# jambo6/online-neural-cdes

Hardware: AMD Instinct MI355X
Metric: solved integration steps/sec (fwd+adjoint) (higher is better)
Workload: dtype f32; 1 GPU; BASELINE cfg2: rectilinear interpolation, rk4 step 1, B=4096 per GPU (global 4096), raw L=200 -> T=399 knots, C=20, H=HH=32, nl=3; step = forward + adjoint backward + Adam; global_batch=4096, seq_len=200, parallelism=dp1

## Files before the change

include/ncde_hip.h:

```cpp
#ifndef NCDE_HIP_H
#define NCDE_HIP_H

#include <stddef.h>
#include <stdint.h>

#ifdef __cplusplus
extern "C" {
#endif

#define NCDE_ABI_VERSION 4
#define NCDE_MAX_LAYERS 8

typedef enum NcdeStatus {
    NCDE_OK = 0,
    NCDE_ERR_INVALID = -1,
    NCDE_ERR_UNSUPPORTED = -2,
    NCDE_ERR_WORKSPACE = -3,
    NCDE_ERR_HIP = -4
} NcdeStatus;

typedef enum NcdeInterp { NCDE_INTERP_LINEAR = 0, NCDE_INTERP_CUBIC = 1, NCDE_INTERP_QUINTIC = 2 } NcdeInterp;

typedef enum NcdeMethod { NCDE_EULER = 0, NCDE_MIDPOINT = 1, NCDE_RK4_38 = 2 } NcdeMethod;

typedef enum NcdeOutput { NCDE_OUT_INTERVAL = 0, NCDE_OUT_KNOTS = 1, NCDE_OUT_TIMES = 2 } NcdeOutput;

#define NCDE_FLAG_AUTO 0u
#define NCDE_FLAG_FORCE_GENERIC 1u
#define NCDE_FLAG_FORCE_FAST 2u
#define NCDE_FLAG_FP32_MFMA 4u
#define NCDE_FLAG_ADJOINT_V1 8u
#define NCDE_FLAG_ADJOINT_V2 16u
#define NCDE_FLAG_ADJOINT_V4 32u
#define NCDE_FLAG_SPLIT_BF16 64u
#define NCDE_FLAG_ADJOINT_SPLIT_FP16 128u
#define NCDE_FLAG_DEBUG_PROFILE 0x100u
#define NCDE_FLAG_NO_COOP 0x400u
#define NCDE_FLAG_COOP_FAULT_INJECT 0x800u
#define NCDE_FLAG_TILED_NS1 0x1000u
#define NCDE_FLAG_TILED_NS2 0x2000u
#define NCDE_FLAG_TILED_NS4 0x4000u
#define NCDE_FLAG_FORCE_TILED 0x8000u

#define NCDE_FLAG_TILED_WINDOW_STEPS(n) (((uint32_t)(n) & 0xFFu) << 16)

typedef struct NcdeProblem {
    int32_t abi_version;
    int32_t batch;
    int32_t n_knots;
    int32_t channels;
    int32_t hidden;
    int32_t interp;
    int32_t method;
    int32_t output;
    uint32_t flags;

    int32_t n_layers;
    int32_t layer_in[NCDE_MAX_LAYERS];
    int32_t layer_out[NCDE_MAX_LAYERS];
    const float* layer_W[NCDE_MAX_LAYERS];
    const float* layer_b[NCDE_MAX_LAYERS];
    const float* Wo;
    const float* bo;

    const float* coeffs;
    int64_t coeffs_stride_b;
    int64_t coeffs_stride_t;

    const float* z0;

    int32_t field_kind;
    int32_t field_input;
    const float* Wg;
    const float* bg;
    const float* Wr;
    const float* br;

    const void* time_plan;
    int32_t n_t_out;
    int32_t n_steps_fwd;
    int32_t n_steps_adj;
    int32_t reserved_;
} NcdeProblem;

typedef enum NcdeFieldKind { NCDE_FIELD_ORIGINAL = 0, NCDE_FIELD_MINIMAL = 1, NCDE_FIELD_GRU = 2 } NcdeFieldKind;
typedef enum NcdeFieldInput { NCDE_INPUT_MATMUL = 0, NCDE_INPUT_EVALUATE = 1, NCDE_INPUT_DERIVATIVE = 2 } NcdeFieldInput;

typedef struct NcdeGrads {
    float* grad_z0;
    float* grad_layer_W[NCDE_MAX_LAYERS];
    float* grad_layer_b[NCDE_MAX_LAYERS];
    float* grad_Wo;
    float* grad_bo;
    float* grad_Wg;
    float* grad_bg;
// ... 102 lines not shown
```

online-neural-cdes_amd/_lib.py:

```python
import ctypes
import os

NCDE_ABI_VERSION = 4
NCDE_MAX_LAYERS = 8

INTERP = {"linear": 0, "cubic": 1, "quintic": 2}
INTERP_PARTS = {"linear": 1, "cubic": 4, "quintic": 6}
METHOD = {"euler": 0, "midpoint": 1, "rk4": 2}
OUT_INTERVAL, OUT_KNOTS, OUT_TIMES = 0, 1, 2
FIELD_KIND = {"original": 0, "minimal": 1, "gru": 2}
FIELD_INPUT = {"matmul": 0, "evaluate": 1, "derivative": 2}
FLAG_AUTO, FLAG_FORCE_GENERIC, FLAG_FORCE_FAST, FLAG_FP32_MFMA, FLAG_ADJOINT_V1, FLAG_ADJOINT_V2 = 0, 1, 2, 4, 8, 16
FLAG_ADJOINT_V4 = 32
FLAG_SPLIT_BF16 = 64
FLAG_NO_COOP = 0x400
FLAG_COOP_FAULT_INJECT = 0x800
FLAG_ADJOINT_SPLIT_FP16 = 128


def FLAG_TILED_WINDOW_STEPS(n):
    return (int(n) & 0xFF) << 16
FLAG_TILED_NS1, FLAG_TILED_NS2, FLAG_TILED_NS4, FLAG_FORCE_TILED = 0x1000, 0x2000, 0x4000, 0x8000

_c_float_p = ctypes.c_void_p


class NcdeProblem(ctypes.Structure):
    _fields_ = [
        ("abi_version", ctypes.c_int32),
        ("batch", ctypes.c_int32),
        ("n_knots", ctypes.c_int32),
        ("channels", ctypes.c_int32),
        ("hidden", ctypes.c_int32),
        ("interp", ctypes.c_int32),
        ("method", ctypes.c_int32),
        ("output", ctypes.c_int32),
        ("flags", ctypes.c_uint32),
        ("n_layers", ctypes.c_int32),
        ("layer_in", ctypes.c_int32 * NCDE_MAX_LAYERS),
        ("layer_out", ctypes.c_int32 * NCDE_MAX_LAYERS),
        ("layer_W", _c_float_p * NCDE_MAX_LAYERS),
        ("layer_b", _c_float_p * NCDE_MAX_LAYERS),
        ("Wo", _c_float_p),
        ("bo", _c_float_p),
        ("coeffs", _c_float_p),
        ("coeffs_stride_b", ctypes.c_int64),
        ("coeffs_stride_t", ctypes.c_int64),
        ("z0", _c_float_p),
        ("field_kind", ctypes.c_int32),
        ("field_input", ctypes.c_int32),
        ("Wg", _c_float_p),
        ("bg", _c_float_p),
        ("Wr", _c_float_p),
        ("br", _c_float_p),
        ("time_plan", ctypes.c_void_p),
        ("n_t_out", ctypes.c_int32),
        ("n_steps_fwd", ctypes.c_int32),
        ("n_steps_adj", ctypes.c_int32),
        ("reserved_", ctypes.c_int32),
    ]


class NcdeTimeSpec(ctypes.Structure):
    _fields_ = [
        ("n_t", ctypes.c_int32),
        ("time_is_f64", ctypes.c_int32),
        ("t", ctypes.POINTER(ctypes.c_double)),
        ("step_size", ctypes.c_double),
        ("knots", ctypes.POINTER(ctypes.c_double)),
    ]


class NcdeTimePlanInfo(ctypes.Structure):
    _fields_ = [
        ("n_t_out", ctypes.c_int32),
# ... 156 lines not shown
```

online-neural-cdes_amd/csrc/ncde_common.h:

```cpp
#pragma once
#include <hip/hip_runtime.h>
#include <stdint.h>

#include "ncde_hip.h"

typedef float f32x4 __attribute__((ext_vector_type(4)));

__device__ __forceinline__ float quintic_eval(const float* p, int cs, float f, bool value) {
    const float bb = p[cs], c2 = p[2 * cs], d3 = p[3 * cs], e4 = p[4 * cs], f5 = p[5 * cs];
    if (value) {
        float inner = 0.25f * e4 + (f5 * f) / 5.0f;
        inner = d3 / 3.0f + inner * f;
        inner = 0.5f * c2 + inner * f;
        inner = bb + inner * f;
        return p[0] + inner * f;
    }
    float inner = e4 + f5 * f;
    inner = d3 + inner * f;
    inner = c2 + inner * f;
    return bb + inner * f;
}

#define NCDE_TILE 16

// ... 7 lines not shown
    const float* coeffs;
    long long cs_b, cs_t;
    const float* z0;
    float* out;
    const float* z_out;
    const float* grad_out;
    float* grad_z0;
    float* gpart;
    int gW_off[NCDE_MAX_LAYERS], gb_off[NCDE_MAX_LAYERS];
    int gWo_off, gbo_off, theta_size;
    int gacc_in_lds;
    float* stages;
    int discrete;
    float* recA;
    float* recB;
    float* recC;
    float* recD;
    int gstride;
    int win_hi, win_lo, resume;
    float* carry;
    int field_kind, field_input;
    int d0;
    int rows;
    const float* Wg;
    const float* bg;
    const float* Wr;
    const float* br;
    int gWg_off, gbg_off, gWr_off, gbr_off;
    const int* plan;
    int n_steps_fwd, n_steps_adj;
    const float* Wo_pk;
    int* fault;
    int only_faulted;
    const float* Wg_pk;
    const unsigned* Wo_bf;
    int wres[NCDE_MAX_LAYERS], wres_o, wres_g, wres_r;
    int tres[NCDE_MAX_LAYERS], tres_o, tres_g;
    int Hr, Cc;
    const unsigned* coop_img;
    float* coop_x;
    float* coop_state;
    unsigned* coop_sync;
    const float* coop_scale;
    int coop_M, coop_G;
    float* recS;
    unsigned* win_max;
    int dw2_parts;
    int dw2_accum;
    int Brec;
    unsigned* coop_status;
    const unsigned* run_if;
    unsigned coop_spin;
    int coop_inject;
};

typedef void (*NcdeKernel)(KArgs);

#define NCDE_PLAN_MAGIC 0x4e43504c
#define NCDE_PLAN_HEADER 8
struct StageDesc {
    int idx;
    float frac;
    float kdt;
};
__host__ __device__ __forceinline__ int plan_step_words(int S) { return 3 + 3 * S; }
__host__ __device__ __forceinline__ int plan_off_fwd() { return NCDE_PLAN_HEADER; }
__host__ __device__ __forceinline__ int plan_off_out(int S, int n_fwd) { return NCDE_PLAN_HEADER + n_fwd * plan_step_words(S); }
__host__ __device__ __forceinline__ int plan_off_adj(int S, int n_fwd, int n_out) { return plan_off_out(S, n_fwd) + 2 * n_out; }
__device__ __forceinline__ bool plan_header_ok(const KArgs& a, int S) {
    const int* h = a.plan;
    return h[0] == NCDE_PLAN_MAGIC && h[1] == S && h[2] == a.n_steps_fwd && h[3] == a.n_steps_adj && h[4] == a.n_out;
}
__device__ __forceinline__ StageDesc plan_stage(const int* step, int j) {
    StageDesc d;
    d.idx = step[3 + 3 * j];
    d.frac = __int_as_float(step[4 + 3 * j]);
    d.kdt = __int_as_float(step[5 + 3 * j]);
    return d;
}

__device__ __forceinline__ int ru4(int x) { return (x + 3) & ~3; }
__device__ __forceinline__ int ru16(int x) { return (x + 15) & ~15; }

__device__ __forceinline__ f32x4 mfma16(float a, float b, f32x4 c) {
    return __builtin_amdgcn_mfma_f32_16x16x4f32(a, b, c, 0, 0, 0);
}

__device__ __forceinline__ float tanh_dev(float x) {
    const float e = __builtin_amdgcn_exp2f(x * 2.8853900817779268f);
    const float r = __builtin_amdgcn_rcpf(e + 1.0f);
    return __builtin_fmaf(-2.0f, r, 1.0f);
}

#define NCDE_TANH_PRESCALE 2.8853900817779268f
__device__ __forceinline__ float tanh_prescaled(float x2l) {
    const float e = __builtin_amdgcn_exp2f(x2l);
    const float r = __builtin_amdgcn_rcpf(e + 1.0f);
    return __builtin_fmaf(-2.0f, r, 1.0f);
}

__device__ __forceinline__ float relu_dev(float x) { return __builtin_amdgcn_fmed3f(x, 0.0f, __builtin_inff()); }

__device__ __forceinline__ int n_stages(int method) { return method == NCDE_RK4_38 ? 4 : (method == NCDE_MIDPOINT ? 2 : 1); }
__device__ __forceinline__ float stage_offset(int method, int j) {
    if (method == NCDE_RK4_38) return j == 0 ? 0.0f : (j == 1 ? 0.333333343267440796f : (j == 2 ? 0.666666686534881592f : 1.0f));
    if (method == NCDE_MIDPOINT) return j == 0 ? 0.0f : 0.5f;
// ... 67 lines not shown
```

online-neural-cdes_amd/csrc/ncde_fast.hip:

```cpp
#include "ncde_fast.h"
#include "ncde_fast4.h"
#include "ncde_fast64.h"
#include "ncde_fast_nl.h"
#include "ncde_fast_c.h"
#include "ncde_fast_fwd3.h"
#include "ncde_fast_plan.h"
#ifndef NCDE_F2_DW_LATE
#define NCDE_F2_DW_LATE 0
#endif
#ifndef NCDE_F2_DXL_BF3
#define NCDE_F2_DXL_BF3 1
#endif
#ifndef NCDE_F2_DWO_EARLY
#define NCDE_F2_DWO_EARLY 0
#endif
#ifndef NCDE_H2_DW_LATE
#define NCDE_H2_DW_LATE 1
#endif
#ifndef NCDE_H2_DWO_EARLY
#define NCDE_H2_DWO_EARLY 0
#endif

#include <cstring>
#include <type_traits>
// ... 1610 lines not shown
    unsigned long long prof[6] = {0, 0, 0, 0, 0, 0}, tlast = 0;
#define NCDE_TICK(k)                                                \
    if constexpr (PROF != 0) {                                      \
        const unsigned long long now_ = __builtin_readcyclecounter(); \
        prof[k] += now_ - tlast;                                    \
        tlast = now_;                                               \
    }
    constexpr int H = 32, HH = 32, NW = 4, HT = 2;
    constexpr int CP = (C + 3) & ~3, CQ = CP / 4, NB = H / 4 / NW;
    constexpr int S = kStages<METHOD>;
    constexpr int NT = 64 * NW;
    constexpr int DXW = INTERP == NCDE_INTERP_LINEAR ? CP : 3 * CP;
    constexpr int EPT = (16 * DXW + NT - 1) / NT;
    constexpr int NTILE = NB * CQ, NBLK = NTILE / 2;
    constexpr int XROWS = H + NL * HH;
    constexpr int NFLAG = NTILE + 2;
    constexpr int HPF = HP != 0 ? 1 : 0, HPC = HP == 1 ? 1 : 0;
    typedef SplitOps<HPF> SF;
    typedef SplitOps<HPC> SO;
    typedef typename SF::T SpF;
    typedef typename SO::T SpT;
    constexpr int NPF = SF::NP, NP = SO::NP;
    if constexpr (HP == 0) {
        if (a.only_faulted && a.fault[blockIdx.x] == 0) return;
    }
    static_assert(NB == 2 && NTILE % 2 == 0, "one 32-row dWo block per cq");
    static_assert(PLAN == 0 || DISC == 0, "the planned discrete backward runs on the batch-tiled family");
    if constexpr (PLAN != 0) {
        if (a.plan == nullptr || !plan_header_ok(a, S)) return;
    }
    const int pw_ = plan_step_words(S);
    const int* padj = PLAN ? a.plan + plan_off_adj(S, a.n_steps_fwd, a.n_out) : nullptr;
    const int n_rsteps = PLAN ? a.n_steps_adj : a.T - 1;
    extern __shared__ __attribute__((aligned(16))) float lds[];
    float* zx = lds;
    float* dxs = zx + 2 * H * 16;
    constexpr int DXR = PLAN ? 2 * S * 16 * CP : 3 * 16 * DXW;
    float* red = dxs + DXR;
    float* boL = red + NW * HH * 16;
    float* tiles = boL + NW * NTILE * 16;
    float* ximg = tiles + NW * NTILE * 256;
    float* dpimg = ximg + 2 * XROWS * 16;
    constexpr int NDP = ((HP == 1 && NCDE_H2_DW_LATE != 0) || (HP == 2 && NCDE_F2_DW_LATE != 0 && INTERP == NCDE_INTERP_LINEAR)) ? 2 : 1;
    constexpr bool DXL3 = HP == 2 && NCDE_F2_DXL_BF3 != 0;
    constexpr bool DWO0_LATE = (HP == 1 && NCDE_H2_DWO_EARLY == 0) || (HP == 2 && NCDE_F2_DWO_EARLY == 0);
    int* flags = reinterpret_cast<int*>(dpimg + NDP * NL * HH * 16);
    float* biasL = reinterpret_cast<float*>(flags + NW * NFLAG);
    unsigned* w1T3 = reinterpret_cast<unsigned*>(biasL + 2 * HT * 16);
    unsigned* w0T3 = w1T3 + HT * NP * 256;
    unsigned* woLo = w0T3 + NW * NP * 256;
    unsigned* w1S3 = woLo + ((HP == 2 && !DXL3) ? 0 : NW * NB * CQ * 256);
    float* amax = reinterpret_cast<float*>(w1S3 + 2 * HT * NPF * 256);
    int* fault_s = reinterpret_cast<int*>(amax + NW);
    float mx = 0.0f;
    float sig = 1.0f;

    const int tid = threadIdx.x, lane = tid & 63;
    const int wave = __builtin_amdgcn_readfirstlane(tid >> 6);
    const bool is_chain = wave < NW;
    const int pw = is_chain ? wave : wave - NW;
    const int s = lane & 15, g = lane >> 4;
    const int b0 = blockIdx.x * NCDE_TILE;
    const int bs = b0 + s;
    const bool valid = bs < a.B;
    float* my_tiles = tiles + pw * NTILE * 256;
    volatile __attribute__((address_space(3))) int* my_flags =
        (volatile __attribute__((address_space(3))) int*)(flags + pw * NFLAG);
    volatile __attribute__((address_space(3))) int* xflag = (volatile __attribute__((address_space(3))) int*)(flags + NTILE);
    const float* boLw = boL + pw * NTILE * 16;

    for (int e = tid; e < NW * NFLAG; e += 512) flags[e] = 0;
    if (tid == 0) *fault_s = 0;
    for (int e = tid; e < NW * NTILE * 16; e += 512) {
        const int r = e & 3, gg = (e >> 2) & 3, rest = e >> 4;
        const int t2 = rest % NTILE, wv = rest / NTILE;
        const int nb = t2 / CQ, cq = t2 - nb * CQ;
        const int h = 4 * (wv * NB + nb) + gg, c = 4 * cq + r;
        boL[e] = c < C ? NCDE_TANH_PRESCALE * a.bo[h * C + c] : 0.0f;
    }
    for (int e = tid; e < 2 * HT * 16; e += 512) {
        const int r = e & 3, gg = (e >> 2) & 3, t = (e >> 4) % HT, layer = e / (16 * HT);
        biasL[e] = (layer == 0 || NL > 1) ? a.b[layer][8 * gg + 4 * t + r] : 0.0f;
    }
    if (tid < 64 * HT) {
        const int l = tid & 63, t = tid >> 6;
        const int unit_out = 8 * ((l & 15) >> 2) + 4 * t + (l & 3);
        float tmp[8];
#pragma unroll
        for (int jj = 0; jj < 8; ++jj) tmp[jj] = NL > 1 ? a.W[1][(8 * (l >> 4) + jj) * HH + unit_out] : 0.0f;
        SO::store(w1T3 + t * NP * 256, l, SO::split(tmp, mx));
    } else if (tid >= 64 * HT + 64 * NW && tid < 64 * HT + 64 * NW + 64 * HT) {
        const int l = tid & 63, t = (tid >> 6) - HT - NW;
        const int unitA = 8 * ((l & 15) >> 2) + 4 * t + (l & 3);
#pragma unroll
        for (int layer = 0; layer < 2; ++layer) {
            float tmp[8];
#pragma unroll
            for (int jj = 0; jj < 8; ++jj) tmp[jj] = (layer == 0 || NL > 1) ? a.W[layer][unitA * HH + 8 * (l >> 4) + jj] : 0.0f;
            SF::store(w1S3 + (layer * HT + t) * NPF * 256, l, SF::split(tmp, mx));
        }
    } else if (tid < 64 * HT + 64 * NW) {
        const int l = tid & 63, wv = (tid >> 6) - HT;
        const int r_own = l & 3;
        const int hrow = 4 * (wv * NB + r_own) + ((l & 15) >> 2);
        float tmp[8];
#pragma unroll
// ... 3 lines not shown

    if (is_chain) {
        u32x4 woHi[NB][CQ], woMid[NB][CQ];
        unsigned* my_woLo = woLo + pw * NB * CQ * 256;
        auto fwd_weights = [&](int layer, int tt) { return SF::load(w1S3 + (layer * HT + tt) * NPF * 256, lane); };
        auto wo_operand = [&](int nb, int cq) {
            SpF As;
            As.hi = woHi[nb][cq];
            if constexpr (HPF != 0) {
                As.lo = woMid[nb][cq];
            } else {
                As.mid = woMid[nb][cq];
                As.lo = *reinterpret_cast<const u32x4*>(my_woLo + ((nb * CQ + cq) * 64 + lane) * 4);
            }
            return As;
        };
#pragma unroll
        for (int nb = 0; nb < NB; ++nb)
#pragma unroll
            for (int cq = 0; cq < CQ; ++cq) {
                const int hA = 4 * (pw * NB + nb) + (s >> 2), cA = 4 * cq + (s & 3);
                float tmp[8];
#pragma unroll
                for (int jj = 0; jj < 8; ++jj) tmp[jj] = cA < C ? NCDE_TANH_PRESCALE * a.Wo[(hA * C + cA) * HH + 8 * g + jj] : 0.0f;
                const SpF sp = SF::split(tmp, mx);
                woHi[nb][cq] = sp.hi;
                if constexpr (HPF != 0) {
                    woMid[nb][cq] = sp.lo;
                } else {
                    woMid[nb][cq] = sp.mid;
                    *reinterpret_cast<u32x4*>(my_woLo + ((nb * CQ + cq) * 64 + lane) * 4) = sp.lo;
                }
            }
        const float* eptr[EPT];
        float eprev[EPT], enext[EPT];
        bool eok[EPT];
#pragma unroll
        for (int q = 0; q < EPT; ++q) {
            const int e = tid + q * NT;
            const int es = e / DXW, ec = e - es * DXW;
            const int part = ec / CP, c = ec - part * CP;
            eok[q] = e < 16 * DXW && c < a.Cc && (b0 + es) < a.B;
            const long long base = (long long)(eok[q] ? b0 + es : 0) * a.cs_b;
            eptr[q] = a.coeffs + base + (INTERP == NCDE_INTERP_LINEAR ? c : (part + 1) * a.Cc + c);
            eprev[q] = 0.0f;
            enext[q] = 0.0f;
        }
        auto stage_load = [&](int piece) {
#pragma unroll
            for (int q = 0; q < EPT; ++q) enext[q] = eok[q] ? eptr[q][(long long)piece * a.cs_t] : 0.0f;
        };
        auto stage_store = [&](int piece) {
            float* dst = dxs + (piece % 3) * 16 * DXW;
#pragma unroll
            for (int q = 0; q < EPT; ++q) {
                const int e = tid + q * NT;
                if (e < 16 * DXW) dst[e] = INTERP == NCDE_INTERP_LINEAR ? eprev[q] - enext[q] : enext[q];
                eprev[q] = enext[q];
            }
        };
        constexpr int EPQ = PLAN ? (S * 16 * CP + NT - 1) / NT : 1;
        float qn[EPQ];
        auto plan_load = [&](const int* pstep) {
#pragma unroll
            for (int q = 0; q < EPQ; ++q) {
                const int e = tid + q * NT;
                const int j = e / (16 * CP), rem = e - j * (16 * CP), es = rem / CP, c = rem - es * CP;
                float v = 0.0f;
                if (e < S * 16 * CP && c < a.Cc && b0 + es < a.B) {
                    const StageDesc sd = plan_stage(pstep, j);
                    const float* p = a.coeffs + (long long)(b0 + es) * a.cs_b + (long long)sd.idx * a.cs_t;
                    if constexpr (INTERP == NCDE_INTERP_LINEAR) {
                        v = p[a.cs_t + c] - p[c];
                        if (sd.kdt != 1.0f) v = v / sd.kdt;
                    } else {
                        const float bb = p[a.Cc + c], cc = p[2 * a.Cc + c], dd = p[3 * a.Cc + c];
                        const float inner = cc + dd * sd.frac;
                        v = bb + inner * sd.frac;
                    }
                }
                qn[q] = v;
            }
        };
        auto plan_store = [&](int buf) {
#pragma unroll
            for (int q = 0; q < EPQ; ++q) {
                const int e = tid + q * NT;
                if (e < S * 16 * CP) dxs[buf * (S * 16 * CP) + e] = qn[q];
            }
        };
        const int p_hi = a.n_pieces - 1;
        if constexpr (PLAN != 0) {
            plan_load(padj);
            plan_store(0);
        } else {
            if (INTERP == NCDE_INTERP_LINEAR) {
#pragma unroll
                for (int q = 0; q < EPT; ++q) eprev[q] = eok[q] ? eptr[q][(long long)(p_hi + 1) * a.cs_t] : 0.0f;
            }
            stage_load(p_hi);
            stage_store(p_hi);
            if (p_hi >= 1) {
                stage_load(p_hi - 1);
                stage_store(p_hi - 1);
            }
        }
        const int last_row = a.n_out - 1;
        float y0[NB], ky1[NB], ky2[NB], a0[NB], ka1[NB], ka2[NB], as_[NB], zreg[8];
        f32x4 znext[2];
        auto rec_fetch = [&](int lin) {
            const float* rp = a.stages + ((long long)lin * a.B + (valid ? bs : 0)) * a.Hr + 8 * g;
// ... 490 lines not shown
                        Aw.lo = *reinterpret_cast<const u32x4*>(my_woTlo + (((t_lo / 2) * HT + tt) * 64 + lane) * 4);
                        mfma_split2(Aw, Bq, accJ[tt], accJx[tt]);
                    }
                }
            } else {
                float bq[t_hi - t_lo][4];
#pragma unroll
                for (int tau = t_lo; tau < t_hi; ++tau)
#pragma unroll
                    for (int r = 0; r < 4; ++r) bq[tau - t_lo][r] = my_tiles[tau * 256 + (4 * g + r) * 16 + s];
#pragma unroll
                for (int tau = t_lo; tau < t_hi; ++tau)
#pragma unroll
                    for (int tt = 0; tt < HT; ++tt)
#pragma unroll
                        for (int r = 0; r < 4; ++r) accJ[tt] = mfma16(woT[tau][tt][r], bq[tau - t_lo][r], accJ[tt]);
            }
        };
        auto rescale_acc = [&]() {
            if constexpr (HPC != 0) {
                if (sig != acc_sig) {
                    const float ratio = sig * h2_inv_scale(acc_sig);
#pragma unroll
                    for (int i = 0; i < NBLK; ++i) {
                        gbo[i] *= ratio;
#pragma unroll
                        for (int q = 0; q < 16; ++q) gWo[i][q] *= ratio;
                    }
#pragma unroll
                    for (int r = 0; r < 4; ++r) { gW1[r] *= ratio; gW0[r] *= ratio; }
                    gb1 *= ratio;
                    gb0 *= ratio;
                    acc_sig = sig;
                }
            }
        };
        int sc = 0;
        float wprev = 0.0f;
        if constexpr (PROF != 0) tlast = __builtin_readcyclecounter();
        for (int n = n_rsteps; n >= 1; --n) {
            const float dtw = PLAN ? __int_as_float(padj[(n_rsteps - n) * pw_]) : 1.0f;
#pragma unroll 1
            for (int j = 0; j < S; ++j) {
                ++sc;
                const int par = sc & 1;
                const float wq = DISC != 0 ? 1.0f : stage_weight(METHOD, j) * dtw;
                if (NDP == 1 && wprev != 0.0f) dw_hidden(par ^ 1, wprev);
                NCDE_TICK(0)
#pragma unroll
                for (int tt = 0; tt < HT; ++tt) accJ[tt] = accJx[tt] = zero4;
                if constexpr (NDP == 1) rescale_acc();
                SpT Bs;
                bool have_bs = false;
#pragma unroll
                for (int blk = 0; blk < NBLK; ++blk) {
                    NCDE_TICK(2)
                    wait_flag(2 * blk + 1, sc);
                    NCDE_TICK(1)
                    if (blk == 0) dxl_tiles(std::integral_constant<int, 0>{}, std::integral_constant<int, 2>{});
                    else if (blk == 1) dxl_tiles(std::integral_constant<int, 2>{}, std::integral_constant<int, 4>{});
                    else if (blk == 2) { if constexpr (NBLK > 2) dxl_tiles(std::integral_constant<int, 4>{}, std::integral_constant<int, 6>{}); }
                    else if (blk == 3) { if constexpr (NBLK > 3) dxl_tiles(std::integral_constant<int, 6>{}, std::integral_constant<int, 8>{}); }
                    else if (blk == 4) { if constexpr (NBLK > 4) dxl_tiles(std::integral_constant<int, 8>{}, std::integral_constant<int, 10>{}); }
                    static_assert(NBLK <= 5, "extend the block dispatch");
                    if (wq != 0.0f && blk == 1 && !DWO0_LATE) {
                        if (!have_bs) {
                            while (__builtin_amdgcn_readfirstlane(*xflag) != sc) __builtin_amdgcn_s_sleep(1);
                            wave_lds_order();
                            Bs = x3_split(par, wq);
                            have_bs = true;
                        }
                        dwo_block(Bs, wq, blk >> 1);
                    }
                }
                NCDE_TICK(3)
#pragma unroll
                for (int tt = 0; tt < HT; ++tt) {
                    if constexpr (HPC != 0) accJ[tt] = h2_combine(accJ[tt], accJx[tt]);
#pragma unroll
                    for (int r = 0; r < 4; ++r) red[pw * HH * 16 + (8 * g + 4 * tt + r) * 16 + s] = accJ[tt][r];
                }
                NCDE_TICK(4)
                __syncthreads();
                if constexpr (NDP == 2) {
                    if (wprev != 0.0f) dw_hidden(par ^ 1, wprev);
                    rescale_acc();
                }
                if (wq != 0.0f) {
                    if (!have_bs) {
                        while (__builtin_amdgcn_readfirstlane(*xflag) != sc) __builtin_amdgcn_s_sleep(1);
                        wave_lds_order();
                        Bs = x3_split(par, wq);
                    }
#pragma unroll
                    for (int blk = 0; blk < NBLK; ++blk)
                        if (blk >= 1 || DWO0_LATE) dwo_block(Bs, wq, blk);

                }
                __syncthreads();
                if constexpr (HPC != 0) {
                    if (j == S - 1) sig = h2_pick_scale(__builtin_fmaxf(__builtin_fmaxf(amax[0], amax[1]), __builtin_fmaxf(amax[2], amax[3])), sig);
                }
                NCDE_TICK(5)
                wprev = wq;
            }
        }
        if (wprev != 0.0f) dw_hidden(sc & 1, wprev);
        if constexpr (PROF != 0) {
            if (lane == 0) {
                unsigned long long* dst = reinterpret_cast<unsigned long long*>(a.out) + ((long long)blockIdx.x * 8 + wave) * 6;
                for (int k = 0; k < 6; ++k) dst[k] = prof[k];
            }
        }
        float* gp = a.gpart + (long long)blockIdx.x * a.theta_size;
        if constexpr (HPC != 0) {
            const float un = h2_inv_scale(acc_sig);
#pragma unroll
            for (int i = 0; i < NBLK; ++i) {
                gbo[i] *= un;
#pragma unroll
                for (int q = 0; q < 16; ++q) gWo[i][q] *= un;
            }
#pragma unroll
            for (int r = 0; r < 4; ++r) { gW1[r] *= un; gW0[r] *= un; }
            gb1 *= un;
            gb0 *= un;
        }
#pragma unroll
        for (int blk = 0; blk < NBLK; ++blk) {
#pragma unroll
            for (int q = 0; q < 16; ++q) {
                const int nb = q >> 3;
                const int gr = 2 * ((q >> 2) & 1) + (lane >> 5), rr = q & 3;
                const int h = 4 * (pw * NB + nb) + gr, c = 4 * blk + rr;
                if (c < C) gp[a.gWo_off + (h * C + c) * HH + (lane & 31)] = gWo[blk][q];
            }
            float v = gbo[blk];
            v += __shfl_xor(v, 32, 64);
            const int i32 = lane & 31;
            const int nb = i32 >> 4, rowt = i32 & 15;
            const int hrow = 4 * (pw * NB + nb) + (rowt >> 2), crow = 4 * blk + (rowt & 3);
            if (lane < 32 && crow < C) gp[a.gbo_off + hrow * C + crow] = v;
        }
#pragma unroll
        for (int r = 0; r < 4; ++r) {
            if constexpr (NL > 1) gp[a.gW_off[1] + (16 * tr + 4 * g + r) * HH + 16 * tc + s] = gW1[r];
            gp[a.gW_off[0] + (16 * tr + 4 * g + r) * H + 16 * tc + s] = gW0[r];
        }
        {
            float v1 = gb1, v0 = gb0;
// ... 85 lines not shown
                                    2 * (H + NL * HH) * 16 + NL * HH * 16 + NW * 2 * NTILE + 2 * (HH / 16) * 16 +
                                    (HH / 16) * (HH / 16) * 256 + NW * (HH / 16) * 256);
}

#ifdef NCDE_DEV_KNOBS
#define NCDE_ADJ3_HP1(NL_, C_, I_, M_, P_, D_) ncde_adj_fast3<NL_, C_, I_, M_, P_, D_, 1>
#define NCDE_ADJ3_HP1_AVAILABLE 1
#else
#define NCDE_ADJ3_HP1(NL_, C_, I_, M_, P_, D_) static_cast<NcdeKernel>(nullptr)
#define NCDE_ADJ3_HP1_AVAILABLE 0
#endif

template <int NL, int C>
NcdeKernel pick_adj3(int interp, int method, int hp) {
#define NCDE_PICK(I, M) \
    if (interp == I && method == M) return hp == 2 ? ncde_adj_fast3<NL, C, I, M, 0, 0, 2> : (hp == 1 ? NCDE_ADJ3_HP1(NL, C, I, M, 0, 0) : ncde_adj_fast3<NL, C, I, M>);
    NCDE_PICK(NCDE_INTERP_LINEAR, NCDE_RK4_38)
    NCDE_PICK(NCDE_INTERP_LINEAR, NCDE_MIDPOINT)
    NCDE_PICK(NCDE_INTERP_LINEAR, NCDE_EULER)
    NCDE_PICK(NCDE_INTERP_CUBIC, NCDE_RK4_38)
    NCDE_PICK(NCDE_INTERP_CUBIC, NCDE_MIDPOINT)
    NCDE_PICK(NCDE_INTERP_CUBIC, NCDE_EULER)
#undef NCDE_PICK
    return nullptr;
}

template <int NL, int C>
NcdeKernel pick_adj3_disc(int interp, int method, int hp) {
#define NCDE_PICK(I, M) \
    if (interp == I && method == M) return hp == 2 ? ncde_adj_fast3<NL, C, I, M, 0, 1, 2> : (hp == 1 ? NCDE_ADJ3_HP1(NL, C, I, M, 0, 1) : ncde_adj_fast3<NL, C, I, M, 0, 1>);
    NCDE_PICK(NCDE_INTERP_LINEAR, NCDE_RK4_38)
    NCDE_PICK(NCDE_INTERP_LINEAR, NCDE_MIDPOINT)
    NCDE_PICK(NCDE_INTERP_LINEAR, NCDE_EULER)
    NCDE_PICK(NCDE_INTERP_CUBIC, NCDE_RK4_38)
    NCDE_PICK(NCDE_INTERP_CUBIC, NCDE_MIDPOINT)
    NCDE_PICK(NCDE_INTERP_CUBIC, NCDE_EULER)
#undef NCDE_PICK
    return nullptr;
}

#endif
template <int NL, int C>
size_t adj3_lds_bytes(int interp, int hp, int plan_stages);
template <int NL, int C>
size_t adj3_lds_bytes(int interp, int hp) { return adj3_lds_bytes<NL, C>(interp, hp, 0); }
template <int NL, int C>
size_t adj3_lds_bytes(int interp, int hp, int plan_stages) {
    constexpr int H = 32, HH = 32, NW = 4, HT = 2, CP = (C + 3) & ~3, CQ = CP / 4, NB = 2, NTILE = NB * CQ;
    const int DXW = interp == NCDE_INTERP_LINEAR ? CP : 3 * CP;
    const int DXR = plan_stages ? 2 * plan_stages * 16 * CP : 3 * 16 * DXW;
    const int NPF = hp ? 2 : 3, NP = hp == 1 ? 2 : 3, NDP = ((hp == 1 && NCDE_H2_DW_LATE) || (hp == 2 && NCDE_F2_DW_LATE && interp == NCDE_INTERP_LINEAR)) ? 2 : 1;
    return sizeof(float) * (size_t)(2 * H * 16 + DXR + NW * HH * 16 + NW * NTILE * 16 + NW * NTILE * 256 +
                                    2 * (H + NL * HH) * 16 + NDP * NL * HH * 16 + NW * (NTILE + 2) + 2 * HT * 16 +
                                    HT * NP * 256 + NW * NP * 256 + ((hp == 2 && !NCDE_F2_DXL_BF3) ? 0 : NW * NB * CQ * 256) + 2 * HT * NPF * 256 + NW + 4);
}

#ifndef NCDE_FAST_KERNELS_ONLY
template <int H, int HH, int C, int NL, int NW>
size_t adj_lds_bytes(int interp) {
    constexpr int CP = (C + 3) & ~3, CQ = CP / 4, HT = HH / 16, NB = H / 4 / NW, NTILE = NB * CQ;
    const int DXW = interp == NCDE_INTERP_LINEAR ? CP : 3 * CP;
    constexpr int PRIV = (H + NL * HH) * 20 + HH * 20;
    return sizeof(float) * (size_t)(2 * H * 16 + 3 * 16 * DXW + NW * HH * 16 + NW * NTILE * HT * 256 + NW * NTILE * 16 + NW * PRIV);
}

struct FastEntry {
    int H, HH, C;
    NcdeKernel (*fwd)(int interp, int method);
    NcdeKernel (*fwd_split)(int interp, int method, int n_layers, int hp);
    bool adjoint;
};
const FastEntry kFast[] = {
    {32, 32, 20, pick_fwd<32, 32, 20, 4>, pick_fwd_bf3<32, 32, 20, 4>, true},
    {64, 64, 4, pick_fwd<64, 64, 4, 4>, pick_fwd_bf3<64, 64, 4, 4>, false},
    {32, 32, 40, pick_fwd<32, 32, 40, 4>, pick_fwd_bf3<32, 32, 40, 4>, false},
};
constexpr int kAdjLayers = 3;

const FastEntry* find_entry(const NcdeProblem* p) {
    if (p->n_layers < 1) return nullptr;
    const int HH = p->layer_out[0];
    for (int l = 1; l < p->n_layers; ++l)
        if (p->layer_out[l] != HH || p->layer_in[l] != HH || p->layer_W[l] != p->layer_W[1] || p->layer_b[l] != p->layer_b[1]) return nullptr;
    for (const FastEntry& e : kFast)
        if (e.H == p->hidden && e.HH == HH && e.C == p->channels) return &e;
    return nullptr;
}

int c_set(const NcdeProblem* p) {
    if (p->hidden != 32 || p->n_layers < 1 || p->n_layers > 4 || p->layer_out[0] != 32 || p->layer_in[0] != 32) return 0;
    if (p->channels != 4 && p->channels != 8 && p->channels != 12) return 0;
    if (p->field_kind != NCDE_FIELD_ORIGINAL || p->field_input != NCDE_INPUT_MATMUL || p->output == NCDE_OUT_TIMES) return 0;
    for (int l = 1; l < p->n_layers; ++l)
        if (p->layer_out[l] != 32 || p->layer_in[l] != 32 || p->layer_W[l] != p->layer_W[1] || p->layer_b[l] != p->layer_b[1]) return 0;
    if (p->n_layers > 1 && (p->layer_W[1] == p->layer_W[0] || p->layer_b[1] == p->layer_b[0])) return 0;
    if (p->flags & (NCDE_FLAG_FP32_MFMA | NCDE_FLAG_ADJOINT_V1 | NCDE_FLAG_ADJOINT_V2 | NCDE_FLAG_ADJOINT_V4 | NCDE_FLAG_ADJOINT_SPLIT_FP16 |
                    NCDE_FLAG_DEBUG_PROFILE | kFlagChainDump)) return 0;
    return p->channels;
}
NcdeKernel c_fwd(int C, int interp, int method, int hp) {
    return C == 4 ? ncde_fast_c4_fwd(interp, method, hp) : (C == 8 ? ncde_fast_c8_fwd(interp, method, hp) : ncde_fast_c12_fwd(interp, method, hp));
}
NcdeKernel c_adj(int C, int nl, int interp, int method, int hp, bool disc) {
    return C == 4 ? ncde_fast_c4_adj(nl, interp, method, hp, disc) : (C == 8 ? ncde_fast_c8_adj(nl, interp, method, hp, disc) : ncde_fast_c12_adj(nl, interp, method, hp, disc));
}
size_t c_adj_lds(int C, int nl, int interp, int hp) {
    return C == 4 ? ncde_fast_c4_adj_lds(nl, interp, hp) : (C == 8 ? ncde_fast_c8_adj_lds(nl, interp, hp) : ncde_fast_c12_adj_lds(nl, interp, hp));
// ... 159 lines not shown
```

online-neural-cdes_amd/csrc/ncde_fastdefs.h:

```cpp
#pragma once
#include "ncde_common.h"
#include "ncde_bf3.h"

namespace {

template <int METHOD>
struct Combine {
    static __device__ __forceinline__ float apply(int j, float k, float& y0, float& k1, float& k2) {
        if constexpr (METHOD == NCDE_RK4_38) {
            if (j == 0) { k1 = k; return y0 + k * 0.333333343267440796f; }
            if (j == 1) { k2 = k; return y0 + (k - k1 * 0.333333343267440796f); }
            if (j == 2) { const float ys = y0 + ((k1 - k2) + k); k2 = k2 + k; return ys; }
            y0 = y0 + ((k1 + 3.0f * k2) + k) * 0.125f;
            return y0;
        } else if constexpr (METHOD == NCDE_MIDPOINT) {
            if (j == 0) return y0 + k * 0.5f;
            y0 = y0 + k;
            return y0;
        } else {
            y0 = y0 + k;
            return y0;
        }
    }
};

__device__ __forceinline__ void wave_lds_order() { asm volatile("" ::: "memory"); }

template <int METHOD> constexpr int kStages = METHOD == NCDE_RK4_38 ? 4 : (METHOD == NCDE_MIDPOINT ? 2 : 1);

__device__ __forceinline__ float relu_bits(float x) {
    const int b = __builtin_bit_cast(int, x);
    return __builtin_bit_cast(float, b > 0 ? b : 0);
}

}
```

online-neural-cdes_amd/csrc/ncde_host.h:

```cpp
#pragma once
#include <mutex>
#include <map>
#include <utility>
#include <hip/hip_runtime.h>

#include <algorithm>
#include <cstring>

#include "ncde_common.h"

struct ReduceSegs {
    int n;
    int off[2 * NCDE_MAX_LAYERS + 6];
    int len[2 * NCDE_MAX_LAYERS + 6];
    float* dst[2 * NCDE_MAX_LAYERS + 6];
};
extern "C" __global__ void ncde_reduce_partials(const float* gpart, int n_part, int theta_size, ReduceSegs segs);

constexpr int kLdsLimit = 160 * 1024;

constexpr uint32_t kFlagChainDump = 0x200u;

inline const char* ncde_dev_env(const char* name) {
#ifdef NCDE_DEV_KNOBS
// ... 54 lines not shown
        }
        if (prevW >= 0) y.gW_off[l] = y.gW_off[prevW];
        else { y.gW_off[l] = off; off += p->layer_out[l] * p->layer_in[l]; }
        if (prevB >= 0) y.gb_off[l] = y.gb_off[prevB];
        else { y.gb_off[l] = off; off += p->layer_out[l]; }
    }
    y.gWo_off = off; off += y.rows * y.dlast;
    y.gbo_off = off; off += y.rows;
    y.gWg_off = y.gbg_off = y.gWr_off = y.gbr_off = 0;
    if (p->field_kind != NCDE_FIELD_ORIGINAL) {
        y.gWg_off = off; off += y.rows * y.dlast;
        y.gbg_off = off; off += y.rows;
    }
    if (p->field_kind == NCDE_FIELD_GRU) {
        y.gWr_off = off; off += y.d0 * y.d0;
        y.gbr_off = off; off += y.d0;
    }
    y.theta_size = off;
    y.n_wg = (p->batch + NCDE_TILE - 1) / NCDE_TILE;
    y.lds_fwd = sizeof(float) * (size_t)(5 * y.HS + 2 * y.DS + y.Cp * 16);
    size_t adj = sizeof(float) * (size_t)(10 * y.HS + ((y.L > 0 ? y.L : 1) + 4) * y.DS + y.Cp * 16 + 4 * 16 * 17);
    y.gacc_in_lds = adj + sizeof(float) * (size_t)y.theta_size <= (size_t)kLdsLimit;
    y.lds_adj = adj + (y.gacc_in_lds ? sizeof(float) * (size_t)y.theta_size : 0);
    return y;
}


inline void fill_kargs(const NcdeProblem* p, const Layout& y, KArgs* a) {
    memset(a, 0, sizeof(*a));
    a->B = p->batch; a->T = p->n_knots; a->C = p->channels; a->H = p->hidden;
    a->interp = p->interp; a->method = p->method; a->output = p->output; a->n_layers = p->n_layers;
    a->n_pieces = p->n_knots - 1;
    a->n_out = p->output == NCDE_OUT_TIMES ? p->n_t_out : (p->output == NCDE_OUT_KNOTS ? p->n_knots : 2);
    if (p->output == NCDE_OUT_TIMES) {
        a->plan = (const int*)p->time_plan;
        a->n_steps_fwd = p->n_steps_fwd;
        a->n_steps_adj = p->n_steps_adj;
    }
    for (int l = 0; l < p->n_layers; ++l) {
        a->din[l] = p->layer_in[l]; a->dout[l] = p->layer_out[l];
        a->W[l] = p->layer_W[l]; a->b[l] = p->layer_b[l];
        a->gW_off[l] = y.gW_off[l]; a->gb_off[l] = y.gb_off[l];
    }
    a->Wo = p->Wo; a->bo = p->bo; a->coeffs = p->coeffs;
    a->cs_b = p->coeffs_stride_b; a->cs_t = p->coeffs_stride_t;
    a->z0 = p->z0;
    a->gWo_off = y.gWo_off; a->gbo_off = y.gbo_off; a->theta_size = y.theta_size;
    a->field_kind = p->field_kind; a->field_input = p->field_input; a->d0 = y.d0; a->rows = y.rows;
    a->Wg = p->Wg; a->bg = p->bg; a->Wr = p->Wr; a->br = p->br;
    a->gWg_off = y.gWg_off; a->gbg_off = y.gbg_off; a->gWr_off = y.gWr_off; a->gbr_off = y.gbr_off;
    a->gacc_in_lds = y.gacc_in_lds;
    a->Hr = p->reserved_ ? (p->reserved_ >> 12) : p->hidden;
    a->Cc = p->reserved_ ? (p->reserved_ & 0xFFF) : p->channels;
}

inline int launch_reduce_partials(const NcdeProblem* p, const Layout& y, const NcdeGrads* g, const float* gpart, int n_part,
                                  hipStream_t st) {
    ReduceSegs segs{};
    int n = 0;
    for (int l = 0; l < p->n_layers; ++l) {
        bool firstW = true, firstB = true;
        for (int q = 0; q < l; ++q) {
            if (p->layer_W[q] == p->layer_W[l]) firstW = false;
            if (p->layer_b[q] == p->layer_b[l]) firstB = false;
        }
        if (firstW) { segs.off[n] = y.gW_off[l]; segs.len[n] = p->layer_out[l] * p->layer_in[l]; segs.dst[n] = g->grad_layer_W[l]; ++n; }
        if (firstB) { segs.off[n] = y.gb_off[l]; segs.len[n] = p->layer_out[l]; segs.dst[n] = g->grad_layer_b[l]; ++n; }
    }
    segs.off[n] = y.gWo_off; segs.len[n] = y.rows * y.dlast; segs.dst[n] = g->grad_Wo; ++n;
    segs.off[n] = y.gbo_off; segs.len[n] = y.rows; segs.dst[n] = g->grad_bo; ++n;
    if (p->field_kind != NCDE_FIELD_ORIGINAL) {
        segs.off[n] = y.gWg_off; segs.len[n] = y.rows * y.dlast; segs.dst[n] = g->grad_Wg; ++n;
        segs.off[n] = y.gbg_off; segs.len[n] = y.rows; segs.dst[n] = g->grad_bg; ++n;
    }
    if (p->field_kind == NCDE_FIELD_GRU) {
        segs.off[n] = y.gWr_off; segs.len[n] = y.d0 * y.d0; segs.dst[n] = g->grad_Wr; ++n;
        segs.off[n] = y.gbr_off; segs.len[n] = y.d0; segs.dst[n] = g->grad_br; ++n;
    }
    segs.n = n;
    for (int i = 0; i < n; ++i)
        if (!segs.dst[i]) return NCDE_ERR_INVALID;
    hipLaunchKernelGGL(ncde_reduce_partials, dim3((y.theta_size + 255) / 256), dim3(256), 0, st, gpart, n_part, y.theta_size, segs);
    return hipGetLastError() == hipSuccess ? NCDE_OK : NCDE_ERR_HIP;
}
```

Baseline: 176.9 million sample-steps/s.

## Skip zero control-increment channel blocks in rectilinear adjoint dX tiles

During the forward stage store, each wave builds a ballot mask of which 4-channel quads of the linear-interpolation increment dX are nonzero and writes it to LDS. The adjoint reads the mask for the current piece and skips dX-weighted tile blocks and the matching dWo accumulations for quads that are entirely zero. Rectilinear interpolation makes many increments zero (time and channel pieces alternate), so a large share of those matmul blocks can be avoided. This adds ballot and LDS overhead, forces the early dWo path off when any quad is skipped, and adds a DENSE_DX flag to turn the skipping off.

```diff
diff --git a/include/ncde_hip.h b/include/ncde_hip.h
--- a/include/ncde_hip.h
+++ b/include/ncde_hip.h
@@ -41,6 +41,8 @@
 #define NCDE_FLAG_TILED_NS2 0x2000u
 #define NCDE_FLAG_TILED_NS4 0x4000u
 #define NCDE_FLAG_FORCE_TILED 0x8000u
+
+#define NCDE_FLAG_DENSE_DX 0x1000000u
 
 #define NCDE_FLAG_TILED_WINDOW_STEPS(n) (((uint32_t)(n) & 0xFFu) << 16)
 
diff --git a/online-neural-cdes_amd/_lib.py b/online-neural-cdes_amd/_lib.py
--- a/online-neural-cdes_amd/_lib.py
+++ b/online-neural-cdes_amd/_lib.py
@@ -21,6 +21,7 @@
 def FLAG_TILED_WINDOW_STEPS(n):
     return (int(n) & 0xFF) << 16
 FLAG_TILED_NS1, FLAG_TILED_NS2, FLAG_TILED_NS4, FLAG_FORCE_TILED = 0x1000, 0x2000, 0x4000, 0x8000
+FLAG_DENSE_DX = 0x1000000
 
 _c_float_p = ctypes.c_void_p
 
diff --git a/online-neural-cdes_amd/csrc/ncde_common.h b/online-neural-cdes_amd/csrc/ncde_common.h
--- a/online-neural-cdes_amd/csrc/ncde_common.h
+++ b/online-neural-cdes_amd/csrc/ncde_common.h
@@ -83,6 +83,7 @@
     const unsigned* run_if;
     unsigned coop_spin;
     int coop_inject;
+    int dense_dx;
 };
 
 typedef void (*NcdeKernel)(KArgs);
diff --git a/online-neural-cdes_amd/csrc/ncde_fast.hip b/online-neural-cdes_amd/csrc/ncde_fast.hip
--- a/online-neural-cdes_amd/csrc/ncde_fast.hip
+++ b/online-neural-cdes_amd/csrc/ncde_fast.hip
@@ -1686,6 +1686,9 @@
     unsigned* w1S3 = woLo + ((HP == 2 && !DXL3) ? 0 : NW * NB * CQ * 256);
     float* amax = reinterpret_cast<float*>(w1S3 + 2 * HT * NPF * 256);
     int* fault_s = reinterpret_cast<int*>(amax + NW);
+    constexpr bool SPARSE = INTERP == NCDE_INTERP_LINEAR && PLAN == 0;
+    constexpr unsigned ALLQ = (1u << CQ) - 1u;
+    unsigned* dxm = reinterpret_cast<unsigned*>(fault_s + 4);
     float mx = 0.0f;
     float sig = 1.0f;
 
@@ -1795,11 +1798,18 @@
         };
         auto stage_store = [&](int piece) {
             float* dst = dxs + (piece % 3) * 16 * DXW;
+            unsigned m = 0;
 #pragma unroll
             for (int q = 0; q < EPT; ++q) {
                 const int e = tid + q * NT;
-                if (e < 16 * DXW) dst[e] = INTERP == NCDE_INTERP_LINEAR ? eprev[q] - enext[q] : enext[q];
+                const float d = INTERP == NCDE_INTERP_LINEAR ? eprev[q] - enext[q] : enext[q];
+                if (e < 16 * DXW) dst[e] = d;
+                if constexpr (SPARSE) m |= !(d == 0.0f) ? 1u << ((e % CP) >> 2) : 0u;
                 eprev[q] = enext[q];
+            }
+            if constexpr (SPARSE) {
+                const unsigned mw = quad_mask_wave<CQ>(m);
+                if (lane == 0) dxm[(piece % 3) * NW + pw] = mw;
             }
         };
         constexpr int EPQ = PLAN ? (S * 16 * CP + NT - 1) / NT : 1;
@@ -2396,8 +2406,7 @@
                 if constexpr (NDP == 1) rescale_acc();
                 SpT Bs;
                 bool have_bs = false;
-#pragma unroll
-                for (int blk = 0; blk < NBLK; ++blk) {
+                auto dxl_block = [&](int blk) __attribute__((always_inline)) {
                     NCDE_TICK(2)
                     wait_flag(2 * blk + 1, sc);
                     NCDE_TICK(1)
@@ -2407,15 +2416,25 @@
                     else if (blk == 3) { if constexpr (NBLK > 3) dxl_tiles(std::integral_constant<int, 6>{}, std::integral_constant<int, 8>{}); }
                     else if (blk == 4) { if constexpr (NBLK > 4) dxl_tiles(std::integral_constant<int, 8>{}, std::integral_constant<int, 10>{}); }
                     static_assert(NBLK <= 5, "extend the block dispatch");
-                    if (wq != 0.0f && blk == 1 && !DWO0_LATE) {
-                        if (!have_bs) {
-                            while (__builtin_amdgcn_readfirstlane(*xflag) != sc) __builtin_amdgcn_s_sleep(1);
-                            wave_lds_order();
-                            Bs = x3_split(par, wq);
-                            have_bs = true;
-                        }
-                        dwo_block(Bs, wq, blk >> 1);
-                    }
+                };
+                auto dwo_early = [&]() __attribute__((always_inline)) {
+                    if (!have_bs) {
+                        while (__builtin_amdgcn_readfirstlane(*xflag) != sc) __builtin_amdgcn_s_sleep(1);
+                        wave_lds_order();
+                        Bs = x3_split(par, wq);
+                        have_bs = true;
+                    }
+                    dwo_block(Bs, wq, 0);
+                };
+                unsigned live = ALLQ;
+                if constexpr (SPARSE) {
+                    const float t = DISC != 0 ? (float)(n - 1) + stage_offset(METHOD, S - 1 - j) : -(-(float)n + stage_offset(METHOD, j));
+                    live = a.dense_dx ? ALLQ : quad_mask_read<NW>(dxm + (piece_index(t, a.n_pieces) % 3) * NW);
+                }
+#pragma unroll
+                for (int blk = 0; blk < NBLK; ++blk) {
+                    if ((live >> blk) & 1u) dxl_block(blk);
+                    if (wq != 0.0f && blk == 1 && !DWO0_LATE && live == ALLQ) dwo_early();
                 }
                 NCDE_TICK(3)
 #pragma unroll
@@ -2438,8 +2457,9 @@
                     }
 #pragma unroll
                     for (int blk = 0; blk < NBLK; ++blk)
-                        if (blk >= 1 || DWO0_LATE) dwo_block(Bs, wq, blk);
-
+                        if (((live >> blk) & 1u) && (blk >= 1 || DWO0_LATE || live != ALLQ)) dwo_block(Bs, wq, blk);
+#pragma unroll
+                    for (int blk = 0; blk < NBLK; ++blk) asm volatile("" ::"v"(gbo[blk]));
                 }
                 __syncthreads();
                 if constexpr (HPC != 0) {
@@ -2631,7 +2651,8 @@
     const int NPF = hp ? 2 : 3, NP = hp == 1 ? 2 : 3, NDP = ((hp == 1 && NCDE_H2_DW_LATE) || (hp == 2 && NCDE_F2_DW_LATE && interp == NCDE_INTERP_LINEAR)) ? 2 : 1;
     return sizeof(float) * (size_t)(2 * H * 16 + DXR + NW * HH * 16 + NW * NTILE * 16 + NW * NTILE * 256 +
                                     2 * (H + NL * HH) * 16 + NDP * NL * HH * 16 + NW * (NTILE + 2) + 2 * HT * 16 +
-                                    HT * NP * 256 + NW * NP * 256 + ((hp == 2 && !NCDE_F2_DXL_BF3) ? 0 : NW * NB * CQ * 256) + 2 * HT * NPF * 256 + NW + 4);
+                                    HT * NP * 256 + NW * NP * 256 + ((hp == 2 && !NCDE_F2_DXL_BF3) ? 0 : NW * NB * CQ * 256) + 2 * HT * NPF * 256 + NW + 4 +
+                                    ((interp == NCDE_INTERP_LINEAR && !plan_stages) ? 3 * NW : 0));
 }
 
 #ifndef NCDE_FAST_KERNELS_ONLY
diff --git a/online-neural-cdes_amd/csrc/ncde_fastdefs.h b/online-neural-cdes_amd/csrc/ncde_fastdefs.h
--- a/online-neural-cdes_amd/csrc/ncde_fastdefs.h
+++ b/online-neural-cdes_amd/csrc/ncde_fastdefs.h
@@ -33,4 +33,19 @@
     return __builtin_bit_cast(float, b > 0 ? b : 0);
 }
 
+template <int CQ>
+__device__ __forceinline__ unsigned quad_mask_wave(unsigned m) {
+    unsigned r = 0;
+#pragma unroll
+    for (int cq = 0; cq < CQ; ++cq) r |= __builtin_amdgcn_ballot_w64(((m >> cq) & 1u) != 0) != 0 ? 1u << cq : 0u;
+    return r;
 }
+template <int NWORDS>
+__device__ __forceinline__ unsigned quad_mask_read(const unsigned* words) {
+    unsigned r = words[0];
+#pragma unroll
+    for (int w = 1; w < NWORDS; ++w) r |= words[w];
+    return __builtin_amdgcn_readfirstlane(r);
+}
+
+}
diff --git a/online-neural-cdes_amd/csrc/ncde_host.h b/online-neural-cdes_amd/csrc/ncde_host.h
--- a/online-neural-cdes_amd/csrc/ncde_host.h
+++ b/online-neural-cdes_amd/csrc/ncde_host.h
@@ -130,6 +130,7 @@
     a->gacc_in_lds = y.gacc_in_lds;
     a->Hr = p->reserved_ ? (p->reserved_ >> 12) : p->hidden;
     a->Cc = p->reserved_ ? (p->reserved_ & 0xFFF) : p->channels;
+    a->dense_dx = (p->flags & NCDE_FLAG_DENSE_DX) ? 1 : 0;
 }
 
 inline int launch_reduce_partials(const NcdeProblem* p, const Layout& y, const NcdeGrads* g, const float* gpart, int n_part,
```

After: 185.5 million sample-steps/s, median of 6. 4.8% higher.
